# Filippo-Galli/Split_and_merge_Gibbs_sampling

Measured on AMD Instinct MI355X. Metric: full Gibbs sweeps/sec (N-point reassign) at N=1M D=128; achieved HBM GB/s, higher is better.
Workload: dtype f64

## Files before the change

include/hdpm.h:

```cpp
#ifndef HDPM_H
#define HDPM_H

#include <stdint.h>

#ifdef __cplusplus
extern "C" {
#endif

#define HDPM_OK          0
#define HDPM_E_VALIDATE  1
#define HDPM_E_GSL       2
#define HDPM_E_PROB      3
#define HDPM_E_WALKER    4
#define HDPM_E_ARG       5
#define HDPM_E_DEVICE    6
#define HDPM_E_NODEVICE  7

typedef struct hdpm_ctx hdpm_ctx;

typedef struct {
    int32_t verbose, m, iterations, L, burnin, t, r;
    int32_t neal8, split_merge, n8_step_size, sam_step_size, thinning;
} hdpm_chain_params;

// ... 10 lines not shown
    double  t_sm_ms, t_sm_scan_ms, t_sm_phi_ms, t_sm_terms_ms;
    int64_t phi_device_calls, phi_device_fallbacks, phi_device_last_status;
    int64_t phi_lookahead_hits, phi_lookahead_copies;
    int64_t pipe_enqueued, pipe_runs, pipe_refused, pipe_recovered;
    int64_t phi_tree_calls, phi_tree_retries;
    int64_t pool_walk_fallbacks;
    int64_t phi_dspec_launched, phi_dspec_used;
    int64_t fpg_launches;
    int64_t phi_sm_device_calls;
    int64_t phi_fallback_status_mask;
    int64_t phi_sm_window_retries;
    int64_t fpg_aborts;
    int64_t exact_mass_launches, exact_lanes_launches;
    int64_t dense_launches;
    int64_t sm_wide_scans, sm_wide_fallbacks;
    int64_t phi_fast_calls, phi_fast_handbacks;
    int64_t labels_mirrored, labels_downloaded;
    int64_t phi_state_direct;
    int64_t phi_chain_launched, phi_chain_used, phi_chain_dropped;
    int64_t pipe_auto, pipe_desync;
    int64_t sm_chain_runs, sm_chain_scans, sm_chain_resumes;
    int64_t pipe_early, pipe_early_ran, pipe_early_off;
    int64_t resolved_by_word;
} hdpm_stats;

int         hdpm_device_count(void);
int         hdpm_ctx_create(int32_t device, hdpm_ctx** out);
void        hdpm_ctx_destroy(hdpm_ctx* ctx);
const char* hdpm_last_error(const hdpm_ctx* ctx);

int hdpm_set_data(hdpm_ctx* ctx, const uint8_t* codes, int32_t n, int32_t d, const int32_t* attrisize,
                  double gamma, const double* v, const double* w);

int hdpm_rng_set_seed(hdpm_ctx* ctx, uint32_t seed);
int hdpm_rng_set_state(hdpm_ctx* ctx, const int32_t* state625);
int hdpm_rng_get_state(const hdpm_ctx* ctx, int32_t* state625);

int hdpm_set_state(hdpm_ctx* ctx, const int32_t* c_i, int32_t K, const double* centers, const double* sigma);
int hdpm_get_state(hdpm_ctx* ctx, int32_t* c_i, int32_t* K, double* centers, double* sigma, int32_t cap);

int hdpm_set_pool(hdpm_ctx* ctx, const double* centers, const double* sigma, int64_t P);
int hdpm_get_pool(hdpm_ctx* ctx, double* centers, double* sigma, int64_t P);
int hdpm_generate_pool(hdpm_ctx* ctx, int64_t P);

int hdpm_neal8_sweep(hdpm_ctx* ctx, int32_t m);

// ... 61 lines not shown
#define HDPM_DBG_COMMIT_FIRST            (1u << 21)
#define HDPM_DBG_NO_PIPE                 (1u << 22)
#define HDPM_DBG_ONE_WAVE_RESOLVER       (1u << 23)
#define HDPM_DBG_FP_LIST_ALL_AFTER_EXACT (1u << 24)
#define HDPM_DBG_FP_ALWAYS               (1u << 25)
#define HDPM_DBG_FP_FROM_STAY            (1u << 26)
#define HDPM_DBG_PHI_WALKS               (1u << 27)
#define HDPM_DBG_POOL_SERIAL_PARSE       (1u << 28)
#define HDPM_DBG_FP_ONE_WG               (1u << 29)
#define HDPM_DBG_FPG_ALWAYS              (1u << 30)
int hdpm_set_debug(hdpm_ctx* ctx, int32_t mode);
int hdpm_get_pool_heads(hdpm_ctx* ctx, uint64_t* out, int64_t P);
#define HDPM_OPT_HIG_LOGSPACE 1
#define HDPM_OPT_PHI_DEVICE 2
#define HDPM_OPT_PIPE_WAIT_US 3
#define HDPM_OPT_CAPTURE_DELAY_US 10
#define HDPM_OPT_FPG_WAIT_US 4
#define HDPM_OPT_FPG_FAIL_AT 5
#define HDPM_OPT_EXACT_KERNEL 6
#define HDPM_OPT_LAT_NEGLIGIBLE 7
#define HDPM_OPT_SM_WIDE_WAIT_US 8
#define HDPM_OPT_SM_CHAIN 9
#define HDPM_OPT_PHI_SD_SCALE 11
int hdpm_set_option(hdpm_ctx* ctx, int32_t option, double value);
int hdpm_get_option(hdpm_ctx* ctx, int32_t option, double* value);
int hdpm_psm_build(hdpm_ctx* ctx, const int32_t* c_trace, int32_t M, int32_t N);
int hdpm_psm_rows(hdpm_ctx* ctx, int32_t row0, int32_t nrows, double* out);
int hdpm_psm_vi_lb(hdpm_ctx* ctx, const int32_t* cls, int32_t ncand, double* out);
int hdpm_trace_build(hdpm_ctx* ctx, const int32_t* c_trace, int32_t M, int32_t N, int64_t table_budget_bytes);
int hdpm_trace_terms(hdpm_ctx* ctx, const int32_t* cls, int32_t ncand, uint64_t* all, uint64_t* same);
int hdpm_trace_losses(hdpm_ctx* ctx, const int32_t* cls, int32_t ncand, double* vi_lb, double* vi,
                      uint64_t* binder_Q, uint64_t* binder_P);
int hdpm_trace_tables(hdpm_ctx* ctx, const int32_t* cls, int32_t ncand, int32_t m0, int32_t nm, uint32_t* out);
int hdpm_trace_distances(hdpm_ctx* ctx, const int32_t* cls, int32_t ncand, double* vi, uint64_t* binder,
                         int32_t* draw_k);
int hdpm_trace_affinity(hdpm_ctx* ctx, const int32_t* cl, int32_t Ka, uint64_t* aff, uint64_t* cross);
#define HDPM_TRACE_GROUPS_DEFAULT 8192
#define HDPM_TRACE_GROUPS_MAX 16384
int hdpm_trace_groups(hdpm_ctx* ctx, int32_t max_groups, int32_t hash_bits, int32_t* U);
int hdpm_trace_group_info(hdpm_ctx* ctx, int32_t* first, int32_t* weight, int32_t* group_of, uint32_t* counts);
int hdpm_trace_avg_tree(hdpm_ctx* ctx, int32_t* merge, double* height);
int hdpm_trace_cut_losses(hdpm_ctx* ctx, int32_t k0, int32_t nk, double* vi_lb, double* vi, uint64_t* binder_A,
                          uint64_t* binder_Q);
int hdpm_trace_cut_labels(hdpm_ctx* ctx, int32_t k, int32_t* cl);
int hdpm_predict_build(hdpm_ctx* ctx, int32_t d, const int32_t* attrisize, double gamma, const int32_t* total_cls,
                       const double* centers, const double* sigmas);
// ... 15 lines not shown
```

split_and_merge_gibbs_sampling_amd/_lib.py:

```python
from __future__ import annotations

import ctypes as C
import enum
import os
import subprocess

import numpy as np

PKG_DIR = os.path.dirname(os.path.abspath(__file__))
LIB_PATH = os.path.join(PKG_DIR, "libhdpm.so")
if os.environ.get("HDPM_LIB_VARIANT"):
    LIB_PATH = os.path.join(PKG_DIR, f"libhdpm_{os.environ['HDPM_LIB_VARIANT']}.so")
CSRC = os.path.join(PKG_DIR, "csrc")

EXPORTS = (
    "hdpm_device_count", "hdpm_ctx_create", "hdpm_ctx_destroy", "hdpm_last_error", "hdpm_set_data",
    "hdpm_rng_set_seed", "hdpm_rng_set_state", "hdpm_rng_get_state", "hdpm_set_state", "hdpm_get_state",
    "hdpm_set_pool", "hdpm_get_pool", "hdpm_generate_pool", "hdpm_neal8_sweep", "hdpm_update_phi",
    "hdpm_compute_loglikelihood", "hdpm_loglik_matrix", "hdpm_restricted_gibbs", "hdpm_logprobgs_c_i",
    "hdpm_split_and_merge", "hdpm_run_markov_chain", "hdpm_get_stats", "hdpm_reset_stats",
    "hdpm_set_debug", "hdpm_synchronize", "hdpm_drop_prepared", "hdpm_init_chain", "hdpm_iteration", "hdpm_iterations", "hdpm_iterations_record", "hdpm_record_take", "hdpm_rng_fill_device",
    "hdpm_get_pool_heads", "hdpm_set_option", "hdpm_get_option", "hdpm_debug_draw", "hdpm_debug_math",
    "hdpm_psm_build", "hdpm_psm_rows", "hdpm_psm_vi_lb",
    "hdpm_trace_build", "hdpm_trace_terms", "hdpm_trace_losses", "hdpm_trace_tables",
    "hdpm_trace_groups", "hdpm_trace_group_info", "hdpm_trace_avg_tree", "hdpm_trace_cut_losses",
    "hdpm_trace_cut_labels", "hdpm_trace_distances", "hdpm_trace_affinity", "hdpm_sm_last_terms",
    "hdpm_predict_build", "hdpm_predict_new", "hdpm_predict_own", "hdpm_predict_loglik",
)

OPT_HIG_LOGSPACE = 1
OPT_PHI_DEVICE = 2
OPT_PIPE_WAIT_US = 3
OPT_FPG_WAIT_US = 4
OPT_FPG_FAIL_AT = 5
OPT_EXACT_KERNEL = 6
OPT_LAT_NEGLIGIBLE = 7
OPT_SM_WIDE_WAIT_US = 8
OPT_SM_CHAIN = 9
OPT_CAPTURE_DELAY_US = 10
OPT_PHI_SD_SCALE = 11


class Debug(enum.IntFlag):
    EXACT_ALL = 1 << 0
    PHASE_TIMES = 1 << 1
    LL_PER_POINT = 1 << 2
    NO_SNAPSHOT = 1 << 3
    RECOUNT = 1 << 4
    TIMELINE = 1 << 5
    HOST_POOL = 1 << 6
    NO_SPEC_PHI = 1 << 7
    NO_PREPARE = 1 << 8
    KERNEL_EVENTS = 1 << 9
    NO_POOL_HEADS = 1 << 10
    EXACT_WAVE = 1 << 11
    NO_BLOCK_MODE = 1 << 12
    BLOCK_MODE_ALWAYS = 1 << 13
    NO_WIDE_PREPASS = 1 << 14
    SWEEP_FIRST = 1 << 15
    SM_HOST_DRAWS = 1 << 16
    NO_PREPASS_AHEAD = 1 << 17
    MARGIN_ONLY = 1 << 18
    PHI_HOST = 1 << 19
# ... 30 lines not shown
    _fields_ = [(n, C.c_int64) for n in (
        "sweeps", "rounds", "restarts", "exact_points", "moves", "checked_rounds", "prepass_points")] + \
        [(n, C.c_double) for n in (
            "t_prepass_ms", "t_resolve_ms", "t_stats_ms", "t_host_phi_ms", "t_rng_ms", "t_loglik_ms",
            "t_exact_ms")] + \
        [(n, C.c_int64) for n in ("pool_calls", "pool_entries", "pool_device_calls")] + \
        [(n, C.c_double) for n in (
            "t_pool_ms", "t_pool_mt_ms", "t_pool_accept_ms", "t_pool_parse_ms", "t_pool_values_ms")] + \
        [(n, C.c_int64) for n in ("phi_spec_runs", "phi_spec_clusters", "prepass_timed", "prepass_timed_points",
                                  "rng_windows", "rng_windows_fresh", "listed_points", "sm_moves")] + \
        [(n, C.c_double) for n in ("t_sm_ms", "t_sm_scan_ms", "t_sm_phi_ms", "t_sm_terms_ms")] + \
        [(n, C.c_int64) for n in ("phi_device_calls", "phi_device_fallbacks", "phi_device_last_status",
                                  "phi_lookahead_hits", "phi_lookahead_copies", "pipe_enqueued", "pipe_runs",
                                  "pipe_refused", "pipe_recovered", "phi_tree_calls", "phi_tree_retries",
                                  "pool_walk_fallbacks", "phi_dspec_launched", "phi_dspec_used",
                                  "fpg_launches", "phi_sm_device_calls", "phi_fallback_status_mask",
                                  "phi_sm_window_retries", "fpg_aborts", "exact_mass_launches",
                                  "exact_lanes_launches", "dense_launches", "sm_wide_scans",
                                  "sm_wide_fallbacks", "phi_fast_calls", "phi_fast_handbacks",
                                  "labels_mirrored", "labels_downloaded", "phi_state_direct",
                                  "phi_chain_launched", "phi_chain_used", "phi_chain_dropped",
                                  "pipe_auto", "pipe_desync", "sm_chain_runs", "sm_chain_scans",
                                  "sm_chain_resumes", "pipe_early", "pipe_early_ran", "pipe_early_off",
                                  "resolved_by_word")]

    def as_dict(self):
        return {k: getattr(self, k) for k, _ in self._fields_}


class SmTerms(C.Structure):
    _fields_ = [("kind", C.c_int32), ("accepted", C.c_int32), ("i1", C.c_int32), ("i2", C.c_int32),
                ("nS", C.c_int32), ("size", C.c_int32 * 3), ("term", C.c_double * 14),
                ("log_prior", C.c_double), ("log_likelihood", C.c_double), ("log_proposal", C.c_double),
                ("log_ratio", C.c_double), ("log_u", C.c_double)]

    def as_dict(self):
        return {"kind": self.kind, "accepted": self.accepted, "i1": self.i1, "i2": self.i2, "nS": self.nS,
                "size": list(self.size), "term": list(self.term), "log_prior": self.log_prior,
                "log_likelihood": self.log_likelihood, "log_proposal": self.log_proposal,
                "log_ratio": self.log_ratio, "log_u": self.log_u}


def build(force: bool = False) -> str:
    srcs = [os.path.join(CSRC, f) for f in os.listdir(CSRC)]
    stale = force or not os.path.exists(LIB_PATH) or \
        max(os.path.getmtime(s) for s in srcs) > os.path.getmtime(LIB_PATH)
    if stale:
# ... 85 lines not shown
```

split_and_merge_gibbs_sampling_amd/csrc/engine.cpp:

```cpp
#include <hip/hip_runtime.h>

#include <algorithm>
#include <cctype>
#include <climits>
#include <atomic>
#include <chrono>
#include <condition_variable>
#include <cstdlib>
#include <functional>
#include <mutex>
#include <pthread.h>
#include <sched.h>
#include <dirent.h>
#include <dlfcn.h>
#include <execinfo.h>
#include <csignal>
#include <unistd.h>
#include <cmath>
#include <cstdio>
#include <cstring>
#include <memory>
#include <string>
#include <thread>
#include <unordered_map>
#include <vector>

#include "../../include/hdpm.h"
#include "host_topology.hpp"
#include "host_util.hpp"
#include "kernels.hpp"
#include "mtjump.hpp"
#include "phi_host.hpp"
#include "pool_host.hpp"
#include "rmath.hpp"
#include "summary_host.hpp"

namespace hdpm {

hipError_t launch_prepass(const PrepassArgs& a, int nblocks, hipStream_t s);
hipError_t launch_cluster_summary(const PrepassArgs& a, hipStream_t s);
hipError_t launch_dense_list(const PrepassArgs& a, hipStream_t s);
hipError_t launch_resolve(const ResolveArgs& a, hipStream_t s);
hipError_t launch_exact_rows(const PrepassArgs& a, int nblocks, hipStream_t s, int* path = nullptr);
size_t resolve_smem_bytes(int scap, int m, int blocks);
size_t resolve_fpg_smem_bytes(int lcap, int m);
int resolve_fpg_max_grid(int lcap, int m);
int warm_sweep_kernels(int lcap, int m);
hipError_t warm_launch_kernels(const PrepassArgs& pa, const ResolveArgs& ra, const int* zero, int* scratch,
                               hipStream_t s);
int device_cus();
hipError_t launch_relabel(int* c, const int* los, int n, const ResolveCtl* ctl, hipStream_t s);
hipError_t launch_finish_sweep(int* counts, int* sol, int* los, int* src, int cap, const ResolveCtl* ctl, int n,
                               hipStream_t s);
hipError_t launch_apply_moves(const int* mlog, const int* mcount, int grid, const uint8_t* codes_t, int d, int nq,
                              int mmax, unsigned int* freq, const ResolveCtl* ctl, int n, int nslots, hipStream_t s);
hipError_t launch_freq_gather(const unsigned int* freq, const int* sol, int Kmax, int fs, unsigned int* out,
                              const ResolveCtl* ctl, int n, hipStream_t s);
// ... 486 lines not shown
    bool valid = false;
    uint64_t pos = 0, epoch = 0;
    int mti = 0;
    int64_t N = 0;
    hipEvent_t ev = nullptr;
    const uint32_t* blk = nullptr;
  } phidev;
  struct PhiSlice {
    PinBuf<uint32_t> buf;
    hipEvent_t ev = nullptr;
    uint64_t s0 = 0, epoch = ~0ull, stamp = 0;
    int64_t words = 0;
    bool valid = false;
  } phis[3];
  uint64_t phis_clock = 0;
  uint64_t look_from = 0;
  int64_t look_words = 0;
  RngWindow win[2];
  int mt_G = 0, mt_bpg = 0;
  DevBuf<uint64_t> d_jpoly;
  DevBuf<uint32_t> d_jidx;
  DevBuf<int> d_joff;
  int64_t cmax = 1 << 16;
  struct PendingAdopt {
    bool active = false;
    hipEvent_t ev = nullptr;
    PinBuf<uint32_t> arr;
    const uint32_t* host_src = nullptr;
    const uint32_t* from_raw = nullptr;
    int mti = 0;
  } pend;
  std::string err;
  hipEvent_t ev[8];

  int n = 0, d = 0, nq = 0, dp = 0, mmax = 0;
  int wb = 1, W = 1, bw = 0;
  bool hig_log = false;
  int Ws = 2;
  double gamma = 0;
  std::vector<int32_t> att;
  std::vector<double> v, w;
  std::vector<uint8_t> codes;
  DevBuf<uint8_t> d_codes_t;
  DevBuf<uint64_t> d_xpk;
  DevBuf<uint64_t> d_xbs;
  DevBuf<double> d_logn;
// ... 295 lines not shown
    }
  }

  void rng_sync() {
    if (!pend.active) return;
    if (pend.from_raw) {
      HIPCHK(hipEventSynchronize(phidev.ev));
      mark("rs.slice");
      for (int i = 0; i < 624; ++i) rng.mt[i] = mt_untemper(pend.from_raw[i]);
    } else {
      HIPCHK(hipEventSynchronize(pend.ev));
      mark("rs.state");
      std::memcpy(rng.mt, pend.host_src ? pend.host_src : pend.arr.p, sizeof(rng.mt));
    }
    rng.mti = pend.mti;
    pend.active = false;
  }
  void rng_drop_pending() { pend.active = false; }

  void size_window(RngWindow& W, int64_t count, int64_t export_after) {
    const int head = W.mti0 >= 624 ? 0 : 624 - W.mti0;
    W.nblocks = count > head ? (int)((count - head + 623) / 624) : 0;
    W.count = count;
    if (W.raw.n < (size_t)count) W.raw.ensure((size_t)count + (size_t)count / 4);
    const size_t aw = (size_t)((count + 623) / 624 + 2) * 624;
    if (W.arrays.n < aw) W.arrays.ensure(aw + aw / 4);
    W.init.ensure(624);
    W.h_init.ensure(624);
    if (!W.done) HIPCHK(hipEventCreateWithFlags(&W.done, hipEventDisableTiming));
    W.export_from = (int)std::max<int64_t>(1, (export_after - head) / 624 - 1);
    W.export_after = export_after;
  }
  void gstream_after_copies() {
    if (pend.ev) HIPCHK(hipStreamWaitEvent(gstream, pend.ev, 0));
    for (auto& sl : phis)
      if (sl.ev) HIPCHK(hipStreamWaitEvent(gstream, sl.ev, 0));
  }
  void run_window(RngWindow& W) {
    ensure_jump(W.count);
    const bool multi = mt_G > 1 && W.count >= (int64_t)mt_G * 624 * 8;
    MtGenArgs a{W.init_src ? W.init_src : W.init.p, W.mti0, W.count, W.raw.p, W.arrays.p, W.nblocks, W.export_from,
                multi ? d_jpoly.p : nullptr, d_jidx.p, d_joff.p, mt_bpg, multi ? mt_G : 1};
    HIPCHK(launch_mt_gen(a, gstream));
    HIPCHK(hipEventRecord(W.done, gstream));
    W.gen++;
    stats.rng_windows++;
    W.valid = true;
  }

  void launch_window(RngWindow& W, int64_t count, int64_t export_after = 0) {
    rng_sync();
    if (rng.mti == 625) {
      uint32_t seed = 4357;
      for (int i = 0; i < 624; i++) {
        rng.mt[i] = seed & 0xffff0000u;
        seed = 69069u * seed + 1u;
        rng.mt[i] |= (seed & 0xffff0000u) >> 16;
        seed = 69069u * seed + 1u;
      }
      rng.mti = 624;
    }
    HIPCHK(hipStreamSynchronize(gstream));
    if (cstream) HIPCHK(hipStreamSynchronize(cstream));
    W.mti0 = rng.mti;
    W.start_pos = rng.pos;
    W.epoch = rng.epoch;
    size_window(W, count, export_after);
    RngWindow& O = (&W == &win[0]) ? win[1] : win[0];
    if (O.raw.n < W.raw.n) O.raw.ensure(W.raw.n);
// ... 9 lines not shown

  void locate(const RngWindow& W, uint64_t target, int64_t* blk, int* mti) const {
    const uint64_t r = target - W.start_pos;
    const uint64_t head = W.mti0 >= 624 ? 0 : 624 - W.mti0;
    if (r < head) {
      *blk = 0;
      *mti = W.mti0 + (int)r;
      return;
    }
    const uint64_t b = 1 + (r - head) / 624, k = (r - head) % 624;
    *blk = (int64_t)(k == 0 ? b - 1 : b);
    *mti = k == 0 ? 624 : (int)k;
    if (*blk != 0 && *blk < W.export_from) throw HipError{hipErrorInvalidValue, "rng window export"};
  }

  void launch_window_from(RngWindow& Wn, RngWindow& Ws, uint64_t target, int64_t count, int64_t export_after) {
    int64_t blk;
    int mti;
    locate(Ws, target, &blk, &mti);
    Wn.mti0 = mti;
    Wn.start_pos = target;
    Wn.epoch = rng.epoch;
    gstream_after_copies();
    size_window(Wn, count, export_after);
    if (blk == 0) {
      HIPCHK(hipMemcpyAsync(Wn.init.p, Ws.init_src ? Ws.init_src : Ws.init.p, 624 * 4, hipMemcpyDeviceToDevice,
                            gstream));
      Wn.init_src = Wn.init.p;
    } else {
      Wn.init_src = Ws.arrays.p + (blk - 1) * 624;
    }
    HIPCHK(hipMemcpyAsync(Wn.h_init.p, Wn.init_src, 624 * 4, hipMemcpyDeviceToHost, gstream));
    run_window(Wn);
  }

  void ensure_jump(int64_t count) {
    const int G = sw::get<sw::MT_WORKGROUPS>();
    if (count < (int64_t)G * 624 * 8) return;
    if (mt_G == G && count <= (int64_t)624 * G * mt_bpg) return;
    const int bpg = (int)((count * 5 / 4 + 624 * G - 1) / (624 * G));
    HIPCHK(hipStreamSynchronize(gstream));
    if (!build_jump(d_jpoly, d_jidx, d_joff, G, bpg)) return;
    mt_G = G;
    mt_bpg = bpg;
  }

  bool build_jump(DevBuf<uint64_t>& jpoly, DevBuf<uint32_t>& jidx, DevBuf<int>& joff, int G, int bpg) {
    static const Poly phi = mt_charpoly();
    if (phi.empty()) return false;
    const uint64_t J = (uint64_t)624 * bpg;
// ... 150 lines not shown
    if (!sl->ev) HIPCHK(hipEventCreateWithFlags(&sl->ev, hipEventDisableTiming));
    HIPCHK(hipStreamWaitEvent(cstream, W.done, 0));
    HIPCHK(hipMemcpyAsync(sl->buf.p, W.raw.p + (s0 - W.start_pos), (size_t)words * 4, hipMemcpyDeviceToHost, cstream));
    HIPCHK(hipEventRecord(sl->ev, cstream));
    sl->valid = true;
    sl->s0 = s0;
    sl->words = words;
    sl->epoch = rng.epoch;
    sl->stamp = ++phis_clock;
    return sl;
  }
  void phi_lookahead() {
    if (!look_from || (debug & HDPM_DBG_NO_LOOKAHEAD)) return;
    const uint64_t from = look_from;
    look_from = 0;
    for (auto& sl : phis)
      if (sl.valid && sl.epoch == rng.epoch && sl.s0 <= from && from + (uint64_t)look_words <= sl.s0 + (uint64_t)sl.words)
        return;
    const RngWindow* X = nullptr;
    for (auto& W : win)
      if (W.valid && W.epoch == rng.epoch && W.start_pos <= from &&
          from + (uint64_t)look_words <= W.start_pos + (uint64_t)W.count && (!X || W.start_pos < X->start_pos))
        X = &W;
    if (X && hipEventQuery(X->done) == hipSuccess) {
      const RngWindow& W = *X;
      {
        const PhiSlice* keep = nullptr;
        for (auto& sl : phis)
          if (phidev.valid && sl.valid && phidev.blk >= sl.buf.p && phidev.blk < sl.buf.p + sl.words) keep = &sl;
        (void)phi_slice_copy(W, from, look_words, keep);
        stats.phi_lookahead_copies++;
      }
    }
  }

  static constexpr int kLead = 8;
  int64_t window_span(int64_t n) const {
    const int64_t cap = (int64_t)1 << 27;
    return std::max(n + cmax, std::min<int64_t>(16 * (n + (1 << 18)), cap));
  }
  const uint32_t* device_draws(int64_t n) {
    RngWindow* W = nullptr;
    for (auto& w : win)
      if (covers(w, rng.pos, n) && (!W || w.start_pos < W->start_pos)) W = &w;
    if (!W) {
      if (win[0].valid || win[1].valid) cmax = std::min<int64_t>(cmax * 2, 1 << 26);
      W = &win[0];
      launch_window(*W, window_span(n), n);
      stats.rng_windows_fresh++;
    }
    mark("dd.window");
    HIPCHK(hipStreamWaitEvent(stream, W->done, 0));
    const uint32_t* p = W->raw.p + (rng.pos - W->start_pos);
    const uint64_t target = rng.pos + n;
    if (!phi_device_prefetch(*W, target, phi_prefetch)) adopt_state_at(*W, target);
    mark("dd.state");
    look_from = target + (uint64_t)n > 624 ? target + (uint64_t)n - 624 : 0;
    look_words = 2 * phi_prefetch + 3 * 624;
    RngWindow* other = (W == &win[0]) ? &win[1] : &win[0];
    const bool ahead = other->valid && other->epoch == rng.epoch && other->start_pos > W->start_pos;
    const uint64_t wend = W->start_pos + (uint64_t)W->count;
    if (!ahead && wend < target + (uint64_t)(kLead * (n + cmax)))
      launch_window_from(*other, *W, target, window_span(n), n);
    return p;
  }

  void tables_for(const uint8_t* cen, const double* sig, uint8_t* out_codes, double* out_tab) const {
    std::memset(out_codes, 0, dp);
    for (int j = 0; j < d; ++j) {
      out_codes[j] = cen[j];
      dhamming_pair(sig[j], att[j], &out_tab[2 * j], &out_tab[2 * j + 1]);
    }
  }

  void bounds_for(const uint8_t* cen, const double* tab, uint64_t* out) const {
    std::memset(out, 0, (size_t)bw * 8);
    long double A = 0.0L, sc = 0.0L;
    double dmax = 0.0, dmin = INFINITY;
    for (int j = 0; j < d; ++j) {
      const unsigned code = cen[j] - 1u;
      for (int b = 0; b < wb; ++b)
        if ((code >> b) & 1u) out[b * Ws + (j >> 6)] |= 1ull << (j & 63);
      A += (long double)tab[2 * j];
      sc += (long double)std::max(std::fabs(tab[2 * j]), std::fabs(tab[2 * j + 1]));
      const double dj = tab[2 * j] - tab[2 * j + 1];
      dmax = std::max(dmax, dj);
// ... 348 lines not shown
  }

  int set_pool(const double* cen, const double* sig, int64_t P_) {
    if (!n) { err = "set_data first"; return kArg; }
    if (P_ <= 0 || P_ > 0x7fffffff) { err = "pool size must be in 1..2^31-1"; return kArg; }
    P = P_;
    pool_on_device = false;
    h_pool_c.resize((size_t)P * d);
    h_pool_s.assign(sig, sig + (size_t)P * d);
    for (size_t q = 0; q < (size_t)P * d; ++q) h_pool_c[q] = (uint8_t)(int)cen[q];
    upload_pool();
    return kOk;
  }

  int generate_pool(int64_t P_) {
    if (!n) { err = "set_data first"; return kArg; }
    if (P_ <= 0 || P_ > 0x7fffffff) { err = "pool size must be in 1..2^31-1"; return kArg; }
    auto t0 = std::chrono::steady_clock::now();
    int st = -1;
    if (!(debug & HDPM_DBG_HOST_POOL) && glibc_selfcheck()) st = generate_pool_device(P_);
    if (st < 0) st = generate_pool_host(P_);
    stats.pool_calls++;
    stats.pool_entries += P_;
    stats.t_pool_ms += std::chrono::duration<double, std::milli>(std::chrono::steady_clock::now() - t0).count();
    return st;
  }

  int generate_pool_host(int64_t P_) {
    P = P_;
    pool_on_device = false;
    h_pool_c.resize((size_t)P * d);
    h_pool_s.resize((size_t)P * d);
    for (int64_t e = 0; e < P; ++e) {
      sample_center_uniform(&h_pool_c[(size_t)e * d]);
      int st = sample_sigma(v.data(), w.data(), &h_pool_s[(size_t)e * d]);
      if (st) { err = "rhig failed in pool generation"; return st; }
    }
    upload_pool();
    return kOk;
  }

  static bool glibc_selfcheck() {
    static const bool ok = [] {
      Rng r;
      r.set_seed(424242u);
      for (int k = 0; k < 200000; ++k) {
// ... 545 lines not shown
    sweep_buffers(track, m);
    __atomic_store_n(&h_pipe.p[q].flag, 0, __ATOMIC_RELEASE);
    __atomic_store_n(&h_pipe.p[q].dev, 0, __ATOMIC_RELEASE);
    h_pipe.p[q].raw = nullptr;
    h_pipe.p[q].raw_dev = nullptr;
    pre.early = false;
    pre.early_raw = nullptr;
    pre.early_went = false;
    const bool dev = !host_spec();
    const uint64_t lo = dev ? dspec.pos : spec.pos;
    const uint64_t hi = lo + (uint64_t)(dev ? dspec.pl.need : 2 * phi_prefetch) + (uint64_t)n * (m + 1);
    int whole = -1;
    for (int k = 0; k < 2; ++k) {
      const RngWindow& w = win[k];
      if (w.valid && w.epoch == rng.epoch && w.start_pos <= lo && hi <= w.start_pos + (uint64_t)w.count &&
          (whole < 0 || w.start_pos < win[whole].start_pos))
        whole = k;
    }
    for (int k = 0; k < 2; ++k) {
      pre.gen[k] = ~0ull;
      const RngWindow& w = win[k];
      if (whole >= 0 ? k == whole
                     : (w.valid && w.epoch == rng.epoch && w.start_pos < hi && lo < w.start_pos + (uint64_t)w.count)) {
        HIPCHK(hipStreamWaitEvent(stream, w.done, 0));
        pre.gen[k] = w.gen;
      }
    }
    PipeAuto au{};
    const bool labels_from_device = record_now && !host_c_valid;
    if (sw::get<sw::PIPE_AUTO>() && dev && pipe_auto && dspec.ran && dspec.fast && dspec.chain && whole >= 0 &&
        !labels_from_device) {
      const RngWindow& w = win[whole];
      au = PipeAuto{dspec.chain, w.raw.p, (int64_t)w.start_pos, w.count, (int64_t)n * (m + 1), 1};
    }
    if (dev) HIPCHK(hipStreamWaitEvent(stream, dspec.ev, 0));
    pipe_seq = next_seq();
    HIPCHK(launch_pipe_wait(&h_pipe.p[q], ctl_at(par), ctl_at(q), n, &d_pipe.p[q], pipe_limit_ticks, stream, au,
                            pipe_seq));
    pre.au = au.on != 0;
    pre.t_enq = std::chrono::steady_clock::now();
    pre.active = true;
    pre.par = q;
    pre.dev = dev;
    pre.buf = dev ? -1 : spec.stage_buf;
    pre.m = m;
    pre.track = track;
// ... 2460 lines not shown
  if (!hdpm::head_fits(ctx->wb, ctx->Ws)) { ctx->err = "no pool-entry heads for this layout"; return HDPM_E_ARG; }
  GUARD({
    HIPCHK(hipMemcpyAsync(out, ctx->d_pool_head.p, (size_t)P * hdpm::head_stride(ctx->wb, ctx->Ws) * 8, hipMemcpyDeviceToHost,
                          ctx->stream));
    HIPCHK(hipStreamSynchronize(ctx->stream));
    return HDPM_OK;
  })
}
int hdpm_get_option(hdpm_ctx* h, int32_t option, double* value) {
  CTX();
  if (!value) return HDPM_E_ARG;
  switch (option) {
    case HDPM_OPT_HIG_LOGSPACE: *value = ctx->hig_log ? 1.0 : 0.0; return HDPM_OK;
    case HDPM_OPT_PHI_DEVICE: *value = (double)ctx->phi_mode; return HDPM_OK;
    case HDPM_OPT_PIPE_WAIT_US: *value = (double)ctx->pipe_limit_ticks * 0.01 * (ctx->pipe_host_check ? 1 : -1); return HDPM_OK;
    case HDPM_OPT_FPG_WAIT_US: *value = (double)ctx->fpg_limit_ticks * 0.01; return HDPM_OK;
    case HDPM_OPT_FPG_FAIL_AT: *value = (double)ctx->fpg_fail_at; return HDPM_OK;
    case HDPM_OPT_EXACT_KERNEL: *value = (double)ctx->exact_pref; return HDPM_OK;
    case HDPM_OPT_LAT_NEGLIGIBLE: *value = ctx->lat_negl; return HDPM_OK;
    case HDPM_OPT_SM_WIDE_WAIT_US: *value = (double)ctx->sm_wide_ticks * 0.01; return HDPM_OK;
    case HDPM_OPT_SM_CHAIN: *value = (double)ctx->sm_chain_mode; return HDPM_OK;
    case HDPM_OPT_CAPTURE_DELAY_US: *value = ctx->capture_delay_us; return HDPM_OK;
    case HDPM_OPT_PHI_SD_SCALE: *value = ctx->phi_sd_scale; return HDPM_OK;
    default:
      ctx->err = "unknown option";
      return HDPM_E_ARG;
  }
}
int hdpm_set_option(hdpm_ctx* h, int32_t option, double value) {
  CTX();
  switch (option) {
    case HDPM_OPT_HIG_LOGSPACE:
      ctx->hig_log = value != 0.0;
      return HDPM_OK;
    case HDPM_OPT_PHI_DEVICE:
      if (!(value == 0.0 || value == 1.0 || value == 2.0 || value == 3.0)) {
        ctx->err = "phi device: 0 host, 1 device, 2 device (general kernels), 3 automatic";
        return HDPM_E_ARG;
      }
      GUARD(ctx->cancel_ahead();)
      ctx->phi_mode = (int)value;
      return HDPM_OK;
    case HDPM_OPT_FPG_WAIT_US:
      if (!(value > 0.0) || !std::isfinite(value)) { ctx->err = "fpg wait limit must be positive"; return HDPM_E_ARG; }
      GUARD(ctx->cancel_ahead();)
      ctx->fpg_limit_ticks = std::max(1LL, (long long)(value * 100.0));
// ... 21 lines not shown
    case HDPM_OPT_SM_CHAIN:
      if (!(value >= 0.0) || !(value <= 1000.0) || value != std::floor(value)) {
        ctx->err = "sm chain: 0 off, 1 on, 2 + 3k / 3 + 3k / 4 + 3k stop at scan k / its updates (testing)";
        return HDPM_E_ARG;
      }
      GUARD(ctx->cancel_ahead();)
      ctx->sm_chain_mode = (int)value;
      return HDPM_OK;
    case HDPM_OPT_PIPE_WAIT_US:
      if (value == 0.0 || !std::isfinite(value)) { ctx->err = "pipe wait limit must be non-zero"; return HDPM_E_ARG; }
      GUARD(ctx->cancel_ahead();)
      ctx->pipe_limit_ticks = std::max(1LL, (long long)(std::fabs(value) * 100.0));
      ctx->pipe_host_check = value > 0;
      return HDPM_OK;
    case HDPM_OPT_CAPTURE_DELAY_US:
      if (!(value >= 0.0) || !(value <= 1e6)) { ctx->err = "capture delay must be in [0, 1e6] us"; return HDPM_E_ARG; }
      ctx->capture_delay_us = value;
      return HDPM_OK;
    case HDPM_OPT_PHI_SD_SCALE:
      if (!(value >= 0.0) || !(value <= 1.0)) { ctx->err = "phi sd scale must be in [0, 1]"; return HDPM_E_ARG; }
      GUARD(ctx->cancel_ahead();)
      ctx->phi_sd_scale = value;
      return HDPM_OK;
    default:
      ctx->err = "unknown option";
      return HDPM_E_ARG;
  }
}
int hdpm_psm_build(hdpm_ctx* h, const int32_t* c_trace, int32_t M, int32_t N) {
  CTX();
  GUARD(return ctx->sum.psm_build(c_trace, M, N);)
}
int hdpm_psm_rows(hdpm_ctx* h, int32_t row0, int32_t nrows, double* out) {
  CTX();
  GUARD(return ctx->sum.psm_rows(row0, nrows, out);)
}
int hdpm_psm_vi_lb(hdpm_ctx* h, const int32_t* cls, int32_t ncand, double* out) {
  CTX();
  GUARD(return ctx->sum.psm_vi_lb(cls, ncand, out);)
}
int hdpm_trace_build(hdpm_ctx* h, const int32_t* c_trace, int32_t M, int32_t N, int64_t table_budget_bytes) {
  CTX();
  GUARD(return ctx->sum.trace_build(c_trace, M, N, table_budget_bytes);)
}
int hdpm_trace_terms(hdpm_ctx* h, const int32_t* cls, int32_t ncand, uint64_t* all, uint64_t* same) {
  CTX();
// ... 101 lines not shown
```

split_and_merge_gibbs_sampling_amd/csrc/switches.hpp:

```cpp
#pragma once
#include <algorithm>
#include <climits>
#include <cstdlib>
#include <cstring>

namespace hdpm::sw {

enum Kind {
  kOn,
  kOff,
  kOnChr,
  kOffChr,
  kSet,
  kInt,
  kIntOr,
  kText,
};
enum When {
  kProcess,
  kContext,
  kLive,
};
struct Switch {
  const char* name;
// ... 12 lines not shown
HDPM_SWITCH(HOST_THREADS, kInt, kContext, "threads of the host pool; <= 0: the hardware's, at most 8")
HDPM_SWITCH(PIN_THREADS, kOn, kContext, "pool workers pinned to the cores of one L3 domain near the GPU")
HDPM_SWITCH(SPIN_US, kInt, kContext, "microseconds an idle pool worker spins before it sleeps", 2000, 0)
HDPM_SWITCH(STREAM_PRIO, kText, kContext, "first character 0: default stream priorities; 2: the sweep's stream low")
HDPM_SWITCH(PHI, kText, kContext, "host | device | device-general | (else) auto: HDPM_OPT_PHI_DEVICE's default")
HDPM_SWITCH(PHI_CHAIN, kOnChr, kProcess, "the next iteration's device update enqueued behind the current speculation")
HDPM_SWITCH(PHI2_GS, kInt, kProcess, "8, 16, 32 or 64 (checked by the caller): the fast update's group size")
HDPM_SWITCH(PHI2_GROUP_THREADS, kIntOr, kProcess, "threads of k_phi2_group's workgroups", 512, 128, 512, 64)
HDPM_SWITCH(PHI2_TREE_THREADS, kIntOr, kProcess, "threads of k_phi2_tree's workgroups; 0: by width", 0, 64, 1024, 64)
HDPM_SWITCH(PHI2_VALUES_WAVES, kIntOr, kProcess, "waves of k_phi2_values' workgroups; 0: by width", 0, 1, 16)
HDPM_SWITCH(PIPE_AUTO, kOnChr, kProcess, "the device's own go for a sweep enqueued behind a fast device update")
HDPM_SWITCH(PIPE_EARLY, kOnChr, kProcess, "the host's early conditional go at the join of the speculated update")
HDPM_SWITCH(RES_WORD, kOnChr, kProcess, "a pipelined round's end taken from its sequence word; 0 keeps the event")
HDPM_SWITCH(DENSE_LIST, kOn, kProcess, "launches that expect most points uncertain list every point")
HDPM_SWITCH(DENSE_DIRECT, kOn, kProcess, "dense launches skip the prepass; 0: they still run it")
HDPM_SWITCH(FPG_MIN, kInt, kProcess, "expected listed points from which launches take k_resolve_fpg", 1024, 1)
HDPM_SWITCH(FP_UNSETTLED_UNIF, kOn, kProcess, "the uniform's certification kept after an unsettled launch; 0: margins")
HDPM_SWITCH(LAT_BOUND, kOn, kProcess, "far latents kept as head bounds by the level-table exact rows; 0: all exact")
HDPM_SWITCH(LV_SPEC, kOn, kProcess, "snapshot draws behind the level-table exact rows (k_snap_draws)")
HDPM_SWITCH(MASS_STATIC, kInt, kProcess, "k_exact_rows_mass: nonzero walks the batches in a fixed order (no claims)")
HDPM_SWITCH(WIDE_WGS, kIntOr, kProcess, "workgroups of k_prepass_wide per CU; 0: by occupancy", 0, 1, 32)
HDPM_SWITCH(WIDE_CLAIM, kInt, kProcess, "k_prepass_wide: nonzero claims chunks from a counter")
HDPM_SWITCH(MT_WORKGROUPS, kIntOr, kProcess, "workgroups of the device stream generator", 256, 2, 4096)
HDPM_SWITCH(SM_CHAIN, kOffChr, kContext, "1: HDPM_OPT_SM_CHAIN starts at 1 (the restricted sampler as a device chain)")
HDPM_SWITCH(SM_WIDE, kOnChr, kProcess, "restricted scans on many CUs (k_sm_scan_wide); 0: one workgroup only")
#undef HDPM_SWITCH

inline int parse(const Switch& s, const char* e) {
  const int v = e ? std::atoi(e) : s.def;
  switch (s.kind) {
    case kOn: return !(e && v == 0);
    case kOff: return e && v == 1;
    case kOnChr: return !(e && e[0] == '0');
    case kOffChr: return e && e[0] == '1';
    case kInt: return e ? std::min(s.hi, std::max(s.lo, v)) : s.def;
    case kIntOr: return v >= s.lo && v <= s.hi && v % s.step == 0 ? v : s.def;
    default: return e != nullptr;
  }
}
template <const Switch& S>
inline int get() {
  static_assert(S.kind != kText, "text switches have their own accessor");
  if constexpr (S.when == kProcess) {
    static const int v = parse(S, std::getenv(S.name));
    return v;
  }
// ... 19 lines not shown
```

split_and_merge_gibbs_sampling_amd/sampler.py:

```python
from __future__ import annotations

import ctypes as C

import numpy as np

from . import _lib
from ._lib import Debug, HdpmError, ptr


def _i32(a):
    return np.ascontiguousarray(a, dtype=np.int32)


def _f64(a):
    return np.ascontiguousarray(a, dtype=np.float64)


class Engine:

    def __init__(self, device: int = 0):
        L = _lib.lib()
        h = C.c_void_p()
        st = L.hdpm_ctx_create(device, C.byref(h))
        if st != 0:
# ... 165 lines not shown
        return out

    def set_phi_device(self, on=True, general: bool = False):
        v = 3.0 if on == "auto" else (2.0 if general else 1.0) if on else 0.0
        self._check(self._L.hdpm_set_option(self._h, _lib.OPT_PHI_DEVICE, v))

    def get_option(self, option: int) -> float:
        v = C.c_double()
        self._check(self._L.hdpm_get_option(self._h, int(option), C.byref(v)))
        return float(v.value)

    @property
    def phi_mode(self) -> str:
        return {0: "host", 1: "device", 2: "device-general", 3: "auto"}[int(self.get_option(_lib.OPT_PHI_DEVICE))]

    def set_pipe_wait_us(self, us: float):
        self._check(self._L.hdpm_set_option(self._h, _lib.OPT_PIPE_WAIT_US, float(us)))

    def set_capture_delay_us(self, us: float):
        self._check(self._L.hdpm_set_option(self._h, _lib.OPT_CAPTURE_DELAY_US, float(us)))

    def set_phi_sd_scale(self, scale: float):
        self._check(self._L.hdpm_set_option(self._h, _lib.OPT_PHI_SD_SCALE, float(scale)))

    def set_fpg_wait_us(self, us: float):
        self._check(self._L.hdpm_set_option(self._h, _lib.OPT_FPG_WAIT_US, float(us)))

    def set_fpg_fail_at(self, k: int):
        self._check(self._L.hdpm_set_option(self._h, _lib.OPT_FPG_FAIL_AT, float(k)))

    def set_exact_kernel(self, which: int):
        self._check(self._L.hdpm_set_option(self._h, _lib.OPT_EXACT_KERNEL, float(which)))

    def set_lat_negligible(self, margin: float):
        self._check(self._L.hdpm_set_option(self._h, _lib.OPT_LAT_NEGLIGIBLE, float(margin)))

    def set_sm_wide_wait_us(self, us: float):
        self._check(self._L.hdpm_set_option(self._h, _lib.OPT_SM_WIDE_WAIT_US, float(us)))

    def set_sm_chain(self, mode: int):
        self._check(self._L.hdpm_set_option(self._h, _lib.OPT_SM_CHAIN, float(mode)))

    def set_hig_logspace(self, on: bool = True):
        self._check(self._L.hdpm_set_option(self._h, _lib.OPT_HIG_LOGSPACE, 1.0 if on else 0.0))

    @staticmethod
# ... 119 lines not shown
```

Baseline: 8685.

## Size RNG generator windows by sweep span and observed draw gaps

```diff
diff --git a/include/hdpm.h b/include/hdpm.h
--- a/include/hdpm.h
+++ b/include/hdpm.h
@@ -56,6 +56,7 @@
     int64_t sm_chain_runs, sm_chain_scans, sm_chain_resumes;
     int64_t pipe_early, pipe_early_ran, pipe_early_off;
     int64_t resolved_by_word;
+    int64_t rng_words_generated, rng_words_reserved, rng_window_max_overlap, rng_window_not_ready;
 } hdpm_stats;
 
 int         hdpm_device_count(void);
@@ -163,6 +164,7 @@
 #define HDPM_OPT_SM_WIDE_WAIT_US 8
 #define HDPM_OPT_SM_CHAIN 9
 #define HDPM_OPT_PHI_SD_SCALE 11
+#define HDPM_OPT_RNG_SPAN 12
 int hdpm_set_option(hdpm_ctx* ctx, int32_t option, double value);
 int hdpm_get_option(hdpm_ctx* ctx, int32_t option, double* value);
 int hdpm_psm_build(hdpm_ctx* ctx, const int32_t* c_trace, int32_t M, int32_t N);
diff --git a/split_and_merge_gibbs_sampling_amd/_lib.py b/split_and_merge_gibbs_sampling_amd/_lib.py
--- a/split_and_merge_gibbs_sampling_amd/_lib.py
+++ b/split_and_merge_gibbs_sampling_amd/_lib.py
@@ -39,6 +39,7 @@
 OPT_SM_CHAIN = 9
 OPT_CAPTURE_DELAY_US = 10
 OPT_PHI_SD_SCALE = 11
+OPT_RNG_SPAN = 12
 
 
 class Debug(enum.IntFlag):
@@ -115,7 +116,8 @@
                                   "phi_chain_launched", "phi_chain_used", "phi_chain_dropped",
                                   "pipe_auto", "pipe_desync", "sm_chain_runs", "sm_chain_scans",
                                   "sm_chain_resumes", "pipe_early", "pipe_early_ran", "pipe_early_off",
-                                  "resolved_by_word")]
+                                  "resolved_by_word", "rng_words_generated", "rng_words_reserved",
+                                  "rng_window_max_overlap", "rng_window_not_ready")]
 
     def as_dict(self):
         return {k: getattr(self, k) for k, _ in self._fields_}
diff --git a/split_and_merge_gibbs_sampling_amd/csrc/engine.cpp b/split_and_merge_gibbs_sampling_amd/csrc/engine.cpp
--- a/split_and_merge_gibbs_sampling_amd/csrc/engine.cpp
+++ b/split_and_merge_gibbs_sampling_amd/csrc/engine.cpp
@@ -33,6 +33,7 @@
 #include "phi_host.hpp"
 #include "pool_host.hpp"
 #include "rmath.hpp"
+#include "rng_windows.hpp"
 #include "summary_host.hpp"
 
 namespace hdpm {
@@ -565,6 +566,7 @@
   DevBuf<uint32_t> d_jidx;
   DevBuf<int> d_joff;
   int64_t cmax = 1 << 16;
+  uint64_t reserved_to = 0, reserved_epoch = ~0ull;
   struct PendingAdopt {
     bool active = false;
     hipEvent_t ev = nullptr;
@@ -906,8 +908,9 @@
     const int head = W.mti0 >= 624 ? 0 : 624 - W.mti0;
     W.nblocks = count > head ? (int)((count - head + 623) / 624) : 0;
     W.count = count;
-    if (W.raw.n < (size_t)count) W.raw.ensure((size_t)count + (size_t)count / 4);
-    const size_t aw = (size_t)((count + 623) / 624 + 2) * 624;
+    const size_t cap = (size_t)window_cap(count);
+    if (W.raw.n < cap) W.raw.ensure(cap + cap / 4);
+    const size_t aw = (size_t)((cap + 623) / 624 + 2) * 624;
     if (W.arrays.n < aw) W.arrays.ensure(aw + aw / 4);
     W.init.ensure(624);
     W.h_init.ensure(624);
@@ -921,7 +924,7 @@
       if (sl.ev) HIPCHK(hipStreamWaitEvent(gstream, sl.ev, 0));
   }
   void run_window(RngWindow& W) {
-    ensure_jump(W.count);
+    ensure_jump(window_cap(W.count));
     const bool multi = mt_G > 1 && W.count >= (int64_t)mt_G * 624 * 8;
     MtGenArgs a{W.init_src ? W.init_src : W.init.p, W.mti0, W.count, W.raw.p, W.arrays.p, W.nblocks, W.export_from,
                 multi ? d_jpoly.p : nullptr, d_jidx.p, d_joff.p, mt_bpg, multi ? mt_G : 1};
@@ -929,6 +932,7 @@
     HIPCHK(hipEventRecord(W.done, gstream));
     W.gen++;
     stats.rng_windows++;
+    stats.rng_words_generated += W.count;
     W.valid = true;
   }
 
@@ -984,10 +988,13 @@
     Wn.start_pos = target;
     Wn.epoch = rng.epoch;
     gstream_after_copies();
+    if (blk == 0) {
+      Wn.init.ensure(624);
+      HIPCHK(hipMemcpyAsync(Wn.init.p, Ws.init_src ? Ws.init_src : Ws.init.p, 624 * 4, hipMemcpyDeviceToDevice,
+                            gstream));
+    }
     size_window(Wn, count, export_after);
     if (blk == 0) {
-      HIPCHK(hipMemcpyAsync(Wn.init.p, Ws.init_src ? Ws.init_src : Ws.init.p, 624 * 4, hipMemcpyDeviceToDevice,
-                            gstream));
       Wn.init_src = Wn.init.p;
     } else {
       Wn.init_src = Ws.arrays.p + (blk - 1) * 624;
@@ -1184,7 +1191,8 @@
       if (W.valid && W.epoch == rng.epoch && W.start_pos <= from &&
           from + (uint64_t)look_words <= W.start_pos + (uint64_t)W.count && (!X || W.start_pos < X->start_pos))
         X = &W;
-    if (X && hipEventQuery(X->done) == hipSuccess) {
+    if (X && hipEventQuery(X->done) != hipSuccess) stats.rng_window_not_ready++;
+    else if (X) {
       const RngWindow& W = *X;
       {
         const PhiSlice* keep = nullptr;
@@ -1196,21 +1204,45 @@
     }
   }
 
-  static constexpr int kLead = 8;
-  int64_t window_span(int64_t n) const {
-    const int64_t cap = (int64_t)1 << 27;
-    return std::max(n + cmax, std::min<int64_t>(16 * (n + (1 << 18)), cap));
+  int rng_span = sw::get<sw::MT_SPAN>();
+  int64_t sweep_n = 0;
+  rngw::GapEstimate gap;
+  int64_t window_span(int64_t n) const { return rngw::window_count(n, gap.est, cmax, rng_span); }
+  int64_t window_cap(int64_t count) const {
+    return std::max(count, rngw::window_count(sweep_n, cmax, cmax, rng_span));
+  }
+  bool pool_jump = false;
+  void note_ready(const RngWindow& W) {
+    if (W.done && hipEventQuery(W.done) != hipSuccess) stats.rng_window_not_ready++;
   }
   const uint32_t* device_draws(int64_t n) {
+    int64_t since = 0;
+    if (rng.epoch == reserved_epoch && rng.pos >= reserved_to) {
+      since = (int64_t)(rng.pos - reserved_to);
+      stats.rng_words_reserved += since;
+      if (!pool_jump) gap.observe(since);
+    } else if (rng.epoch == reserved_epoch) {
+      stats.rng_words_reserved -= (int64_t)(reserved_to - rng.pos);
+    } else {
+      sweep_n = 0;
+      gap.reset(0);
+    }
+    sweep_n = std::max(sweep_n, n);
     RngWindow* W = nullptr;
     for (auto& w : win)
       if (covers(w, rng.pos, n) && (!W || w.start_pos < W->start_pos)) W = &w;
     if (!W) {
-      if (win[0].valid || win[1].valid) cmax = std::min<int64_t>(cmax * 2, 1 << 26);
+      if (rng.epoch == reserved_epoch && reserved_to && !pool_jump) cmax = std::min<int64_t>(cmax * 2, 1 << 26);
       W = &win[0];
-      launch_window(*W, window_span(n), n);
+      launch_window(*W, window_span(sweep_n), n);
       stats.rng_windows_fresh++;
-    }
+    } else {
+      note_ready(*W);
+    }
+    pool_jump = false;
+    reserved_epoch = rng.epoch;
+    stats.rng_words_reserved += n;
+    reserved_to = rng.pos + (uint64_t)n;
     mark("dd.window");
     HIPCHK(hipStreamWaitEvent(stream, W->done, 0));
     const uint32_t* p = W->raw.p + (rng.pos - W->start_pos);
@@ -1222,8 +1254,12 @@
     RngWindow* other = (W == &win[0]) ? &win[1] : &win[0];
     const bool ahead = other->valid && other->epoch == rng.epoch && other->start_pos > W->start_pos;
     const uint64_t wend = W->start_pos + (uint64_t)W->count;
-    if (!ahead && wend < target + (uint64_t)(kLead * (n + cmax)))
-      launch_window_from(*other, *W, target, window_span(n), n);
+    const rngw::Plan pl =
+        rngw::plan_next(W->start_pos, W->count, target, sweep_n, gap.est, cmax, rng_span, rngw::kLead, ahead);
+    if (pl.launch) {
+      stats.rng_window_max_overlap = std::max<int64_t>(stats.rng_window_max_overlap, (int64_t)(wend - pl.start));
+      launch_window_from(*other, *W, pl.start, pl.count, n);
+    }
     return p;
   }
 
@@ -1618,6 +1654,7 @@
     if (st < 0) st = generate_pool_host(P_);
     stats.pool_calls++;
     stats.pool_entries += P_;
+    pool_jump = true;
     stats.t_pool_ms += std::chrono::duration<double, std::milli>(std::chrono::steady_clock::now() - t0).count();
     return st;
   }
@@ -2209,6 +2246,7 @@
       const RngWindow& w = win[k];
       if (whole >= 0 ? k == whole
                      : (w.valid && w.epoch == rng.epoch && w.start_pos < hi && lo < w.start_pos + (uint64_t)w.count)) {
+        note_ready(w);
         HIPCHK(hipStreamWaitEvent(stream, w.done, 0));
         pre.gen[k] = w.gen;
       }
@@ -4715,6 +4753,7 @@
     case HDPM_OPT_SM_CHAIN: *value = (double)ctx->sm_chain_mode; return HDPM_OK;
     case HDPM_OPT_CAPTURE_DELAY_US: *value = ctx->capture_delay_us; return HDPM_OK;
     case HDPM_OPT_PHI_SD_SCALE: *value = ctx->phi_sd_scale; return HDPM_OK;
+    case HDPM_OPT_RNG_SPAN: *value = (double)ctx->rng_span; return HDPM_OK;
     default:
       ctx->err = "unknown option";
       return HDPM_E_ARG;
@@ -4782,6 +4821,14 @@
       GUARD(ctx->cancel_ahead();)
       ctx->phi_sd_scale = value;
       return HDPM_OK;
+    case HDPM_OPT_RNG_SPAN:
+      if (!(value >= 0.0) || !(value <= (double)hdpm::rngw::kSpanMax) || value != std::floor(value)) {
+        ctx->err = "rng span: sweeps per generator window, 1..64, or 0 for the default";
+        return HDPM_E_ARG;
+      }
+      GUARD(ctx->cancel_ahead();)
+      ctx->rng_span = value == 0.0 ? hdpm::sw::get<hdpm::sw::MT_SPAN>() : (int)value;
+      return HDPM_OK;
     default:
       ctx->err = "unknown option";
       return HDPM_E_ARG;
diff --git a/split_and_merge_gibbs_sampling_amd/csrc/rng_windows.hpp b/split_and_merge_gibbs_sampling_amd/csrc/rng_windows.hpp
--- /dev/null
+++ b/split_and_merge_gibbs_sampling_amd/csrc/rng_windows.hpp
@@ -0,0 +1,46 @@
+#pragma once
+#include <algorithm>
+#include <cstdint>
+
+namespace hdpm::rngw {
+
+constexpr int kBlock = 624;
+constexpr int kLead = 8;
+constexpr int kSpanMax = 64;
+constexpr int64_t kCap = (int64_t)1 << 27;
+
+inline int64_t overlap(int64_t n, int64_t cmax) { return n + cmax + 2 * kBlock; }
+inline int64_t advance(int64_t n, int64_t gap, int64_t cmax, int span) {
+  return std::max<int64_t>((int64_t)span * (n + std::min(gap, cmax)), 2 * kBlock);
+}
+inline int64_t window_count(int64_t n, int64_t gap, int64_t cmax, int span) {
+  const int64_t ov = overlap(n, cmax);
+  return std::max(ov, std::min(advance(n, gap, cmax, span) + ov, kCap));
+}
+inline int lead_of(int span, int lead = kLead) { return std::max(1, std::min(lead, span / 2)); }
+
+struct GapEstimate {
+  int64_t est = 0;
+  void reset(int64_t guess) { est = guess; }
+  void observe(int64_t gap) { est = std::max(gap, est - est / 8); }
+};
+
+struct Plan {
+  bool launch = false;
+  uint64_t start = 0;
+  int64_t count = 0;
+};
+inline Plan plan_next(uint64_t wstart, int64_t wcount, uint64_t target, int64_t n, int64_t gap, int64_t cmax, int span,
+                      int lead, bool later) {
+  Plan p;
+  const uint64_t wend = wstart + (uint64_t)wcount;
+  const int64_t ov = overlap(n, cmax);
+  const uint64_t notice = (uint64_t)std::max<int64_t>((int64_t)lead_of(span, lead) * (n + cmax), ov);
+  if (later || target > wend || wend - target >= notice) return p;
+  p.launch = true;
+  p.count = window_count(n, gap, cmax, span);
+  p.start = wcount >= ov + n ? wend - (uint64_t)ov : target;
+  return p;
+}
+
+}
diff --git a/split_and_merge_gibbs_sampling_amd/csrc/switches.hpp b/split_and_merge_gibbs_sampling_amd/csrc/switches.hpp
--- a/split_and_merge_gibbs_sampling_amd/csrc/switches.hpp
+++ b/split_and_merge_gibbs_sampling_amd/csrc/switches.hpp
@@ -58,6 +58,7 @@
 HDPM_SWITCH(WIDE_WGS, kIntOr, kProcess, "workgroups of k_prepass_wide per CU; 0: by occupancy", 0, 1, 32)
 HDPM_SWITCH(WIDE_CLAIM, kInt, kProcess, "k_prepass_wide: nonzero claims chunks from a counter")
 HDPM_SWITCH(MT_WORKGROUPS, kIntOr, kProcess, "workgroups of the device stream generator", 256, 2, 4096)
+HDPM_SWITCH(MT_SPAN, kIntOr, kContext, "sweeps of draws per generator window: HDPM_OPT_RNG_SPAN's default", 16, 1, 64)
 HDPM_SWITCH(SM_CHAIN, kOffChr, kContext, "1: HDPM_OPT_SM_CHAIN starts at 1 (the restricted sampler as a device chain)")
 HDPM_SWITCH(SM_WIDE, kOnChr, kProcess, "restricted scans on many CUs (k_sm_scan_wide); 0: one workgroup only")
 #undef HDPM_SWITCH
diff --git a/split_and_merge_gibbs_sampling_amd/sampler.py b/split_and_merge_gibbs_sampling_amd/sampler.py
--- a/split_and_merge_gibbs_sampling_amd/sampler.py
+++ b/split_and_merge_gibbs_sampling_amd/sampler.py
@@ -211,6 +211,9 @@
 
     def set_phi_sd_scale(self, scale: float):
         self._check(self._L.hdpm_set_option(self._h, _lib.OPT_PHI_SD_SCALE, float(scale)))
+
+    def set_rng_span(self, sweeps: int):
+        self._check(self._L.hdpm_set_option(self._h, _lib.OPT_RNG_SPAN, float(sweeps)))
 
     def set_fpg_wait_us(self, us: float):
         self._check(self._L.hdpm_set_option(self._h, _lib.OPT_FPG_WAIT_US, float(us)))
```

New measurement: 8149. -6.2%, worse.
